# Rose-STL-Lab/spherical-dyffusion

Hardware: AMD Instinct MI355X
Metric: forecast-steps/sec (180x360, 63ch), 25-member ensemble DYffusion sampling, whole job (higher is better)
Workload: dtype f32 tensors; every GEMM-class kernel (1x1 convs, fused MLP, Legendre analysis/synthesis, dhconv) as 3-pass split-f16 MFMA with f32 accumulation; FFT / norms / pointwise in f32 (statistics f64); 1 GPU; 25-member ensemble x horizon-6 DYffusion sampling pass (6 forecaster + 10 interpolator SFNO forwards, dropout stream on, AR feedback), 180x360, 63 state + 2 forcing channels, embed 256, 8 blocks; horizon=6, relayed_members=0, parallelism=members of one initial condition sharded over GPUs, no data-path collective

## Files before the change

spherical-dyffusion_amd/csrc/common.h:

```cpp
#pragma once
#include <hip/hip_runtime.h>
#include <stdint.h>
#include <atomic>
#include <cmath>
#include <type_traits>

#include "../../include/sdy_amd.h"

#define SDY_HIP_TRY(expr)                       \
  do {                                          \
    hipError_t _e = (expr);                     \
    if (_e != hipSuccess) return (int)_e;       \
  } while (0)

#define SDY_TRY(expr)             \
  do {                            \
    int _r = (expr);              \
    if (_r != SDY_OK) return _r;  \
  } while (0)

static inline int sdy_launch_status() {
  hipError_t e = hipGetLastError();
  return e == hipSuccess ? SDY_OK : (int)e;
}

constexpr int SDY_MAX_DEVICES = 64;
static inline int sdy_current_device(int* dev) {
  SDY_HIP_TRY(hipGetDevice(dev));
  return (*dev >= 0 && *dev < SDY_MAX_DEVICES) ? SDY_OK : SDY_ERR_ARG;
}
inline int sdy_cu_count(int* n_cu) {
  static std::atomic<int> cache[SDY_MAX_DEVICES] = {};
  int dev = 0;
  SDY_TRY(sdy_current_device(&dev));
  int v = cache[dev].load(std::memory_order_relaxed);
  if (!v) {
    SDY_HIP_TRY(hipDeviceGetAttribute(&v, hipDeviceAttributeMultiprocessorCount, dev));
    cache[dev].store(v, std::memory_order_relaxed);
  }
  *n_cu = v;
  return SDY_OK;
}
int sdy_flags_ptr(unsigned** flags);
enum { SDY_RANGE_CONV = 0, SDY_RANGE_MLP = 1, SDY_RANGE_DHCONV = 2, SDY_RANGE_LEG_ANALYSIS = 3, SDY_RANGE_LEG_SYNTHESIS = 4 };
int sdy_headroom_ptr(int slot, unsigned** word);
struct SdyOncePerDevice {
  std::atomic<bool> done[SDY_MAX_DEVICES] = {};
  int slot(std::atomic<bool>** flag) {
    int dev = 0;
    SDY_TRY(sdy_current_device(&dev));
    *flag = &done[dev];
    return SDY_OK;
  }
};

constexpr int SDY_MAP_MAX = 128;
struct SdyImgMap {
  int on;
  unsigned char idx[SDY_MAP_MAX];
};
__host__ __device__ __forceinline__ int sdy_img(const SdyImgMap& m, int j) { return m.on ? (int)m.idx[j] : j; }
static inline int sdy_img_map_fill(SdyImgMap& m, const unsigned char* rows, int n) {
  m.on = 0;
  for (int i = 0; i < SDY_MAP_MAX; ++i) m.idx[i] = 0;
  if (!rows) return SDY_OK;
  if (n > SDY_MAP_MAX) return SDY_ERR_UNSUPPORTED;
  m.on = 1;
  for (int i = 0; i < n; ++i) m.idx[i] = rows[i];
  return SDY_OK;
}

typedef float f32x4 __attribute__((ext_vector_type(4)));
template <int B, int E, class F>
__device__ __forceinline__ void sdy_static_for(F&& f) {
  if constexpr (B < E) {
    f(std::integral_constant<int, B>{});
    sdy_static_for<B + 1, E>(f);
  }
}
typedef float sdy_f32x2 __attribute__((ext_vector_type(2)));
typedef _Float16 sdy_f16x2 __attribute__((ext_vector_type(2)));
typedef _Float16 sdy_f16x8 __attribute__((ext_vector_type(8)));
__device__ __forceinline__ void sdy_split8(const float* v, sdy_f16x8& hi, sdy_f16x8& lo) {
#pragma unroll
  for (int e = 0; e < 8; e += 2) {
    const sdy_f32x2 x = {v[e], v[e + 1]};
    const sdy_f16x2 h = __builtin_convertvector(x, sdy_f16x2);
    const sdy_f32x2 r = x - __builtin_convertvector(h, sdy_f32x2);
    const sdy_f16x2 l = __builtin_convertvector(r, sdy_f16x2);
    hi[e] = h[0]; hi[e + 1] = h[1];
    lo[e] = l[0]; lo[e + 1] = l[1];
  }
}
__device__ __forceinline__ void sdy_split8(const float* v, sdy_f16x8& hi, sdy_f16x8& lo, float& amax) {
#pragma unroll
  for (int e = 0; e < 8; e += 2) amax = __builtin_fmaxf(amax, __builtin_fmaxf(__builtin_fabsf(v[e]), __builtin_fabsf(v[e + 1])));
  sdy_split8(v, hi, lo);
}
#ifndef SDY_ACT_SX
#define SDY_ACT_SX 16.0f
#endif
constexpr int SDY_GROUP = 2 * 64;
static inline float sdy_h3_absmax(const float* w, size_t n) {
  float mx = 0.f;
  for (size_t i = 0; i < n; ++i) mx = std::fmax(mx, std::fabs(w[i]));
  return mx;
}
static inline float sdy_h3_scale(float absmax) {
  if (!(absmax > 0.f) || !std::isfinite(absmax)) return 1.0f;
  int e;
  std::frexp(absmax, &e);
  return std::ldexp(1.0f, 13 - e);
}
static inline void sdy_h3_split(float v, _Float16& hi, _Float16& lo) {
// ... 229 lines not shown
```

spherical-dyffusion_amd/csrc/conv_h3.hip:

```cpp
#include <cmath>
#include <cstdlib>
#include <type_traits>
#include <vector>

#include "common.h"

namespace {

constexpr int CE = 256;
constexpr int CTN = 64;
constexpr int CKMAX = 384;
constexpr int CRING = 4;
constexpr float CSX = SDY_ACT_SX;
constexpr int CSTAT_BYTES = CE * 2 * 8;
#ifndef SDY_CONV_STAMP_T0
#define SDY_CONV_STAMP_T0 2
#endif

template <int KBLK, int NW>
struct ConvCfg {
  static_assert(NW == 4 || NW == 8, "4 or 8 waves");
  static constexpr int NT = 64 * NW;
  static constexpr int MT = 8 / NW;
  static constexpr int RS = 4 * NW;
  static constexpr int OC = (8 * KBLK + RS - 1) / RS;
  static constexpr int RPT = 64 / NW;
  static constexpr int PPI = (8 * OC + RPT - 1) / RPT;
  static constexpr int KROW = KBLK <= 4 ? 256 : 384;
  static constexpr int KSW = KROW / 16;
  static constexpr int GPK = 4 * MT;
  static constexpr int GPW = MT * KSW;
  static constexpr int WGS = NW == 4 ? 2 : 1;
  static constexpr int TILE_BYTES = 2 * CTN * KROW * 2;
  static constexpr int LDS_BYTES = TILE_BYTES + CSTAT_BYTES + CE * 4 + SDY_GELU_TAB_BYTES;
};
#ifndef SDY_CONV_GELU_TAB
#define SDY_CONV_GELU_TAB 1
#endif

struct ConvParams {
  const float* x; long x_bs;
  const float* pa; const float* pd;
  const sdy_f16x8* w;
  const float* bias;
  const float* add; long add_bs; int add_mode;
  int act;
  float* out; long out_bs;
  int out_tiled;
  double* stats;
  int HW, B;
  int Cin;
  float out_scale;
  unsigned* flags;
  unsigned* head;
  const float* gelu_tab;
  SdyImgMap xmap;
  unsigned long long* stamps;
};

__device__ __forceinline__ int cv_swz(int px) { return (px & 15) ^ (((px >> 4) & 1) * 3); }
template <int KROW>
__device__ __forceinline__ int cv_off(int px, int c) { return px * KROW + (((c & ~15) | ((c ^ cv_swz(px)) & 15)) << 3); }

template <int KBLK, int NW, bool WS = false>
__global__ __launch_bounds__(64 * NW, NW == 4 ? 2 : 1) void conv_h3_kernel(const ConvParams p) {
  using G = ConvCfg<KBLK, NW>;
  static_assert(!WS || (KBLK == 4 && NW == 8), "weight-stationary: 256 input channels on 8 waves");
  constexpr int RING = WS ? G::KSW : CRING;
  constexpr int CMT = G::MT, CRS = G::RS, COC = G::OC, CRPT = G::RPT, KROW = G::KROW, CGPK = G::GPK, CGPW = G::GPW;
  __shared__ __attribute__((aligned(16))) unsigned char smem[G::LDS_BYTES];
  _Float16* Xs_hi = reinterpret_cast<_Float16*>(smem);
  _Float16* Xs_lo = Xs_hi + CTN * KROW;
  float* Os = reinterpret_cast<float*>(smem);

  const int tid = threadIdx.x, lane = tid & 63, wave = tid >> 6;
  auto Cin = [&] { return WS ? CE : p.Cin; };
  auto add_mode = [&] { return WS ? 1 : p.add_mode; };
  auto act = [&] { return WS ? 1 : p.act; };
  int h = lane >> 5, l31 = lane & 31;
  int q0 = tid & 15, o0 = tid >> 4;
  const int tpi = (p.HW + CTN - 1) / CTN;
  const int ntiles = tpi * p.B;
  const int t_per = (ntiles + (int)gridDim.x - 1) / (int)gridDim.x;
  const int t_begin = (int)blockIdx.x * t_per;
  const int t_end = (t_begin + t_per < ntiles) ? t_begin + t_per : ntiles;

  sdy_f16x8 r_hi[RING], r_lo[RING];
  constexpr int CGROUP_BYTES = SDY_GROUP * (int)sizeof(sdy_f16x8);
  const int uwave = __builtin_amdgcn_readfirstlane(wave);
  const char* const wbase = reinterpret_cast<const char*>(p.w) +
                            (WS ? (size_t)((uwave >> 1) * 2 * G::KSW + (uwave & 1)) * CGROUP_BYTES : (size_t)uwave * CGPW * CGROUP_BYTES);
  unsigned woff = (unsigned)lane * 16u;
#pragma unroll
  for (int s = 0; s < RING; ++s) {
    r_hi[s] = sdy_ring_ld(wbase, woff, 0);
    r_lo[s] = sdy_ring_ld(wbase, woff, CGROUP_BYTES / 2);
    woff += (WS ? 2 : 1) * CGROUP_BYTES;
  }
  constexpr int NWIN = KBLK * CMT;
  if (!WS && NWIN == 1) woff -= CRING * CGROUP_BYTES;

  double* Ss = reinterpret_cast<double*>(smem + G::TILE_BYTES);
  float* Bs = reinterpret_cast<float*>(smem + G::TILE_BYTES + CSTAT_BYTES);
  if (tid < CE) {
    Bs[tid] = p.bias ? p.bias[tid] / p.out_scale : 0.0f;
    Ss[2 * tid] = 0.0; Ss[2 * tid + 1] = 0.0;
  }
  float* Gt = reinterpret_cast<float*>(smem + G::TILE_BYTES + CSTAT_BYTES + CE * 4);
  const unsigned gt_base = (unsigned)(uintptr_t)Gt;
  const bool tab_gelu = SDY_CONV_GELU_TAB && act() == 1;
  if (tab_gelu) gelu_tab_to_lds(Gt, p.gelu_tab, tid, G::NT, 1.0f / SDY_GELU_SX);
  const float os_scale = tab_gelu ? p.out_scale * SDY_GELU_WS : p.out_scale;

  f32x4 xr[COC][8], addv[CRPT];
  auto img = [&](const float* base, long bs, int t) { return base + (long)(t / tpi) * bs; };
  auto ximg = [&](int t) { return p.x + (long)sdy_img(p.xmap, t / tpi) * p.x_bs; };
  auto lane_col = [&](int t) {
    const int nn = (t % tpi) * CTN + 4 * q0;
    return nn < p.HW ? nn : 0;
  };
  const float* addsrc = p.add ? p.add : p.out;
  const long addsrc_bs = p.add ? p.add_bs : p.out_bs;
  if (t_begin < t_end) {
    const float* xz = ximg(t_begin);
    const unsigned xo = (unsigned)(8 * o0 * p.HW + lane_col(t_begin)) * 4u;
#pragma unroll
    for (int oc = 0; oc < COC; ++oc)
#pragma unroll
      for (int e = 0; e < 8; ++e) {
        const int ch = 8 * (o0 + CRS * oc) + e;
        xr[oc][e] = f32x4{0.f, 0.f, 0.f, 0.f};
        if (WS || ch < Cin()) xr[oc][e] = sdy_ld16s(xz + (long)(8 * CRS * oc + e) * p.HW, xo);
      }
  }

  for (int tile = t_begin; tile < t_end; ++tile) {
    asm volatile("" : "+v"(l31), "+v"(h), "+v"(q0), "+v"(o0));
    const int tile_it = tile - t_begin;
    auto stamp = [&](int i) {
      if (SDY_STAMPS_ON && p.stamps && blockIdx.x == 3 && tid == 0 && tile_it >= SDY_CONV_STAMP_T0 && tile_it < SDY_CONV_STAMP_T0 + 4)
        p.stamps[(tile_it - SDY_CONV_STAMP_T0) * 8 + i] = __builtin_amdgcn_s_memtime();
    };
    stamp(0);
    const int z = tile / tpi;
    const int zx = sdy_img(p.xmap, z);
    const int n0 = (tile - z * tpi) * CTN;
    const bool full = n0 + CTN <= p.HW;

    {
      float amax = 0.0f;
      const bool ok = full || (n0 + 4 * q0 < p.HW);
#pragma unroll
      for (int oc = 0; oc < COC; ++oc) {
        const int c0 = 8 * (o0 + CRS * oc);
        if (8 * CRS * oc + 8 * CRS > KROW && c0 >= KROW) continue;
        float av[8], dv[8];
        if (p.pa) {
          const f32x4 a0 = *reinterpret_cast<const f32x4*>(p.pa + (long)zx * CE + c0);
          const f32x4 a1 = *reinterpret_cast<const f32x4*>(p.pa + (long)zx * CE + c0 + 4);
          const f32x4 d0 = *reinterpret_cast<const f32x4*>(p.pd + (long)zx * CE + c0);
          const f32x4 d1 = *reinterpret_cast<const f32x4*>(p.pd + (long)zx * CE + c0 + 4);
#pragma unroll
          for (int e = 0; e < 4; ++e) {
            av[e] = a0[e] * CSX; av[e + 4] = a1[e] * CSX;
            dv[e] = d0[e] * CSX; dv[e + 4] = d1[e] * CSX;
          }
        } else {
#pragma unroll
          for (int e = 0; e < 8; ++e) { av[e] = CSX; dv[e] = 0.f; }
        }
#pragma unroll
        for (int pp = 0; pp < 4; ++pp) {
          sdy_f16x8 vh, vl;
          float v[8];
#pragma unroll
          for (int e = 0; e < 8; ++e) v[e] = (ok && (WS || c0 + e < Cin())) ? fmaf(xr[oc][e][pp], av[e], dv[e]) : 0.0f;
          sdy_split8(v, vh, vl, amax);
          const int off = cv_off<KROW>(4 * q0 + pp, o0 + CRS * oc);
          *reinterpret_cast<sdy_f16x8*>(Xs_hi + off) = vh;
          *reinterpret_cast<sdy_f16x8*>(Xs_lo + off) = vl;
        }
      }
      sdy_flag_range(p.flags, amax, p.head);
    }
    __syncthreads();
    stamp(1);
    const int col = n0 + 4 * q0;
    const bool c_ok = full || col < p.HW;
    const unsigned ro = (unsigned)(o0 * p.HW + (c_ok ? col : 0)) * 4u;
    const unsigned ro_out = p.out_tiled ? (unsigned)(o0 * CTN + 4 * q0) * 4u : ro;
    const int out_rs = p.out_tiled ? CTN : p.HW;
    const int tnext = (tile + 1 < t_end) ? tile + 1 : tile;
    const float* xz_next = ximg(tnext);
    const unsigned xo_next = (unsigned)(8 * o0 * p.HW + lane_col(tnext)) * 4u;
    if constexpr (WS) {
      const float* az = img(p.add, p.add_bs, tile);
#pragma unroll
      for (int i = 0; i < CRPT; ++i) addv[i] = sdy_ld16s(az + (long)(CRS * i) * p.HW, ro);
      __builtin_amdgcn_sched_barrier(0);
    }
    stamp(2);
    f32x16 acc[CMT][2];
#pragma unroll
    for (int mi = 0; mi < CMT; ++mi)
#pragma unroll
      for (int r4 = 0; r4 < 4; ++r4) {
        const f32x4 b4 = *reinterpret_cast<const f32x4*>(Bs + 32 * (CMT * wave + mi) + 8 * r4 + 4 * h);
#pragma unroll
        for (int j = 0; j < 2; ++j)
#pragma unroll
          for (int r = 0; r < 4; ++r) acc[mi][j][4 * r4 + r] = b4[r];
      }
    auto ld_b = [&](int ks, sdy_f16x8* bh, sdy_f16x8* bl) {
#pragma unroll
      for (int j = 0; j < 2; ++j) {
        const int off = cv_off<KROW>(32 * j + l31, 2 * ks + h);
        bh[j] = *reinterpret_cast<const sdy_f16x8*>(Xs_hi + off);
        bl[j] = *reinterpret_cast<const sdy_f16x8*>(Xs_lo + off);
      }
    };
    if constexpr (WS) {
      sdy_f16x8 bh[2][2], bl[2][2];
      ld_b(0, bh[0], bl[0]);
      sdy_static_for<0, G::KSW>([&](auto ks_c) {
        constexpr int ks = decltype(ks_c)::value, c = ks & 1;
        if constexpr (ks + 1 < G::KSW) ld_b(ks + 1, bh[c ^ 1], bl[c ^ 1]);
#pragma unroll
        for (int j = 0; j < 2; ++j) SDY_CROSS_TERM(acc[0][j] = __builtin_amdgcn_mfma_f32_32x32x16_f16(r_lo[ks], bh[c][j], acc[0][j], 0, 0, 0));
#pragma unroll
        for (int j = 0; j < 2; ++j) SDY_CROSS_TERM(acc[0][j] = __builtin_amdgcn_mfma_f32_32x32x16_f16(r_hi[ks], bl[c][j], acc[0][j], 0, 0, 0));
#pragma unroll
        for (int j = 0; j < 2; ++j) acc[0][j] = __builtin_amdgcn_mfma_f32_32x32x16_f16(r_hi[ks], bh[c][j], acc[0][j], 0, 0, 0);
        __builtin_amdgcn_sched_barrier(0);
      });
    } else {
#pragma unroll
    for (int kb = 0; kb < KBLK; ++kb) {
#pragma unroll
      for (int i = 0; i < 4; ++i) {
        const int ks = 4 * kb + i;
        sdy_f16x8 bh[2], bl[2];
        ld_b(ks, bh, bl);
#pragma unroll
        for (int mi = 0; mi < CMT; ++mi) {
          const int g = kb * CGPK + CMT * i + mi;
          const int s = g % CRING;
#pragma unroll
          for (int j = 0; j < 2; ++j) SDY_CROSS_TERM(acc[mi][j] = __builtin_amdgcn_mfma_f32_32x32x16_f16(r_lo[s], bh[j], acc[mi][j], 0, 0, 0));
#pragma unroll
          for (int j = 0; j < 2; ++j) SDY_CROSS_TERM(acc[mi][j] = __builtin_amdgcn_mfma_f32_32x32x16_f16(r_hi[s], bl[j], acc[mi][j], 0, 0, 0));
#pragma unroll
          for (int j = 0; j < 2; ++j) acc[mi][j] = __builtin_amdgcn_mfma_f32_32x32x16_f16(r_hi[s], bh[j], acc[mi][j], 0, 0, 0);
          r_hi[s] = sdy_ring_ld(wbase, woff, 0);
          r_lo[s] = sdy_ring_ld(wbase, woff, CGROUP_BYTES / 2);
          woff += CGROUP_BYTES;
          if ((g + CRING + 1) % (NWIN * CRING) == 0) woff -= NWIN * CRING * CGROUP_BYTES;
          __builtin_amdgcn_sched_barrier(0);
        }
      }
    }
    }

    stamp(3);
    if constexpr (WS) {
      static_assert(!WS || COC == 1, "one channel octet per thread");
#pragma unroll
      for (int e = 0; e < 8; ++e) xr[0][e] = sdy_ld16s(xz_next + (long)e * p.HW, xo_next);
      __builtin_amdgcn_sched_barrier(0);
    } else {
      const float* az = img(addsrc, addsrc_bs, tile);
#pragma unroll
      for (int i = 0; i < CRPT; ++i) addv[i] = p.add ? sdy_ld16s(az + (long)(CRS * i) * p.HW, ro) : f32x4{0.f, 0.f, 0.f, 0.f};
    }
    __syncthreads();
    stamp(4);
#pragma unroll
    for (int mi = 0; mi < CMT; ++mi)
#pragma unroll
      for (int j = 0; j < 2; ++j)
#pragma unroll
        for (int r = 0; r < 16; ++r) {
          const int row = 32 * (CMT * wave + mi) + (r & 3) + 8 * (r >> 2) + 4 * h;
          Os[row * CTN + 32 * j + l31] = acc[mi][j][r] * os_scale;
        }
    __syncthreads();
    stamp(5);
    {
      float* oz = p.out + (long)z * p.out_bs + (p.out_tiled ? (long)(tile - z * tpi) * (CE * CTN) : 0L);
#pragma unroll
      for (int i = 0; i < CRPT; ++i) {
        f32x4 v = *reinterpret_cast<const f32x4*>(Os + (o0 + CRS * i) * CTN + 4 * q0);
        if (tab_gelu) {
          if (add_mode() == 1) v = addv[i] * SDY_GELU_WS + v;
          v = f32x4{gelu_tab16(v.x, gt_base), gelu_tab16(v.y, gt_base), gelu_tab16(v.z, gt_base), gelu_tab16(v.w, gt_base)};
        } else {
        if (add_mode() == 1) v += addv[i];
        if (act() == 1) {
          const sdy_gf2 g0 = gelu_erf2(sdy_gf2{v.x, v.y}), g1 = gelu_erf2(sdy_gf2{v.z, v.w});
          v = f32x4{g0.x, g0.y, g1.x, g1.y};
        }
        }
        if (add_mode() == 2) v += addv[i];
        if (c_ok) sdy_st16s(oz + (long)(CRS * i) * out_rs, ro_out, v);
#pragma unroll
        for (int k = 0; k < G::PPI; ++k) {
          const int piece = G::PPI * i + k, oc = piece >> 3, e = piece & 7;
          if (oc < COC) {
            const int ch = 8 * (o0 + CRS * oc) + e;
            if constexpr (!WS)
              if (ch < Cin()) xr[oc][e] = sdy_ld16s(xz_next + (long)(8 * CRS * oc + e) * p.HW, xo_next);
          }
        }
        if (p.stats) {
          const float s1 = row16_sum(c_ok ? sdy_quad_sum(v) : 0.0f);
          const float s2 = row16_sum(c_ok ? sdy_quad_sumsq(v) : 0.0f);
          if (q0 == 0) {
            double* st = Ss + 2 * (o0 + CRS * i);
            __hip_atomic_fetch_add(st, (double)s1, __ATOMIC_RELAXED, __HIP_MEMORY_SCOPE_WORKGROUP);
            __hip_atomic_fetch_add(st + 1, (double)s2, __ATOMIC_RELAXED, __HIP_MEMORY_SCOPE_WORKGROUP);
          }
        }
      }
    }
    stamp(6);
    {
      const int nt = tile + 1;
      if (p.stats && (nt >= t_end || nt / tpi != z)) {
        __syncthreads();
        if (tid < CE) {
          double* st = p.stats + ((long)z * CE + tid) * 2;
          __hip_atomic_fetch_add(st, Ss[2 * tid], __ATOMIC_RELAXED, __HIP_MEMORY_SCOPE_AGENT);
          __hip_atomic_fetch_add(st + 1, Ss[2 * tid + 1], __ATOMIC_RELAXED, __HIP_MEMORY_SCOPE_AGENT);
          Ss[2 * tid] = 0.0; Ss[2 * tid + 1] = 0.0;
        }
      }
    }
    stamp(7);
    __syncthreads();
  }
}

}

#if SDY_STAMPS_ON
static unsigned long long* g_cstamps = nullptr;
SDY_DEBUG_EXPORT int sdy_conv256_h3_debug_stamps(unsigned long long* host64) {
  if (!g_cstamps || !host64) return SDY_ERR_STATE;
  SDY_HIP_TRY(hipDeviceSynchronize());
  SDY_HIP_TRY(hipMemcpy(host64, g_cstamps, 64 * sizeof(unsigned long long), hipMemcpyDeviceToHost));
  return SDY_OK;
}
#endif

extern "C" int sdy_conv256_h3_supported(int Cin, int Cout) { return (Cin >= 1 && Cin <= CKMAX && Cout == CE) ? 1 : 0; }

static void conv_layout(int Cin, int* nw, int* ksw, int* mt) {
  const int kblk = (Cin + 63) / 64;
  *nw = kblk <= 4 ? 4 : 8;
  *ksw = kblk <= 4 ? 16 : 24;
  *mt = 8 / *nw;
}

extern "C" size_t sdy_conv256_h3_pack_bytes_cin(int Cin) {
  int nw, ksw, mt;
  conv_layout(Cin < 1 ? 1 : Cin, &nw, &ksw, &mt);
  return (size_t)nw * mt * ksw * SDY_GROUP * sizeof(sdy_f16x8);
}
extern "C" size_t sdy_conv256_h3_pack_bytes(void) { return sdy_conv256_h3_pack_bytes_cin(CE); }

extern "C" int sdy_conv256_h3_pack_cin(const float* w_host, int Cin, void* dev, float* scale) {
  if (!w_host || !dev || !scale || Cin < 1 || Cin > CKMAX) return SDY_ERR_ARG;
  const float s = sdy_h3_scale(sdy_h3_absmax(w_host, (size_t)CE * Cin));
  int nw, ksw, mt;
  conv_layout(Cin, &nw, &ksw, &mt);
  const size_t gh = (size_t)SDY_GROUP * 8;
  std::vector<_Float16> buf((size_t)nw * mt * ksw * gh);
  _Float16* d = buf.data();
  for (int w = 0; w < nw; ++w)
    for (int ks = 0; ks < ksw; ++ks)
      for (int mi = 0; mi < mt; ++mi, d += gh)
        sdy_h3_put_group(d, s, [&](int r, int k) {
          const int kk = 16 * ks + k;
          return kk < Cin ? w_host[(size_t)(32 * (mt * w + mi) + r) * Cin + kk] : 0.0f;
        });
  SDY_HIP_TRY(hipMemcpy(dev, buf.data(), buf.size() * sizeof(_Float16), hipMemcpyHostToDevice));
  *scale = s;
  return SDY_OK;
}
extern "C" int sdy_conv256_h3_pack(const float* w_host, void* dev, float* scale) {
  return sdy_conv256_h3_pack_cin(w_host, CE, dev, scale);
}
// ... 59 lines not shown
```

spherical-dyffusion_amd/csrc/mlp_h3.hip:

```cpp
#include <cstdlib>
#include <vector>
#include <cmath>
#include <type_traits>

#include "common.h"

typedef const sdy_f16x8 __attribute__((address_space(1)))* wptr_t;
typedef _Float16 f16x4 __attribute__((ext_vector_type(4)));

namespace {

constexpr int ME = 256;
constexpr int MH = 512;
constexpr int TN = 64;
constexpr int HC = 128;
constexpr int NCH = MH / HC;
constexpr int KS1 = ME / 16;
constexpr int KSC = HC / 16;
constexpr int RING = 16;
constexpr int NGROUPS = NCH * 2 * RING;
static_assert(KS1 == RING && 2 * KSC == RING, "ring slot = index inside a block");
constexpr float SX = SDY_ACT_SX;

struct MlpParams {
// ... 41 lines not shown
  const int t_per = (ntiles + (int)gridDim.x - 1) / (int)gridDim.x;
  const int t_begin = (int)blockIdx.x * t_per;
  const int t_end = (t_begin + t_per < ntiles) ? t_begin + t_per : ntiles;
  int z = 0, zo = 0, n0 = 0;
  bool full = true;

  sdy_f16x8 r_hi[RING], r_lo[RING];
  auto wbase_of = [&](int ln) { return (wptr_t)(p.w + (size_t)wave * (NGROUPS + RING) * SDY_GROUP + ln); };
  wptr_t wp = wbase_of(lane);
#pragma unroll
  for (int s = 0; s < RING; ++s) {
    r_hi[s] = wp[s * SDY_GROUP];
    r_lo[s] = wp[s * SDY_GROUP + 64];
  }
  wp += RING * SDY_GROUP;

  int q0 = tid & 15, o0 = tid >> 4;
  f32x4 xr[2][8];
  const float* pf_base = nullptr;
  const float* res_base = nullptr;
  unsigned pf_off = 0u;
  int pf_rs = 0;
  auto prefetch_setup = [&](int t) {
    const int zz = t / tpi, nn = (t - zz * tpi) * TN;
    const bool ok = nn + 4 * q0 < p.HW;
    pf_base = p.x + (long)zz * p.x_bs + (p.x_tiled ? (long)(t - zz * tpi) * (ME * TN) : 0L);
    pf_rs = p.x_tiled ? TN : p.HW;
    pf_off = p.x_tiled ? (unsigned)(8 * o0 * TN + 4 * q0) * 4u : (unsigned)(8 * o0 * p.HW + (ok ? nn + 4 * q0 : 0)) * 4u;
  };
  auto prefetch_piece = [&](int piece) {
    const int oc = piece >> 3, e = piece & 7;
    xr[oc][e] = sdy_ld16s(pf_base + (long)(8 * 16 * oc + e) * pf_rs, pf_off);
  };
  auto prefetch_x = [&](int t) {
    const int zz = t / tpi, nn = (t - zz * tpi) * TN;
    const bool ok = nn + 4 * q0 < p.HW;
    const float* xz = p.x + (long)zz * p.x_bs + (p.x_tiled ? (long)(t - zz * tpi) * (ME * TN) : 0L);
    const int rs = p.x_tiled ? TN : p.HW;
    const unsigned xo = p.x_tiled ? (unsigned)(8 * o0 * TN + 4 * q0) * 4u : (unsigned)(8 * o0 * p.HW + (ok ? nn + 4 * q0 : 0)) * 4u;
#pragma unroll
    for (int oc = 0; oc < 2; ++oc)
#pragma unroll
      for (int e = 0; e < 8; ++e) xr[oc][e] = sdy_ld16s(xz + (long)(8 * 16 * oc + e) * rs, xo);
  };
  auto load_coeffs = [&](int zz) {
    const int t = 64 * wave + (int)__builtin_amdgcn_mbcnt_hi(~0u, __builtin_amdgcn_mbcnt_lo(~0u, 0u));
    const long c = (long)zz * ME + t, co = (long)sdy_img(p.omap, zz) * ME + t;
    Cf[t] = p.pa ? p.pa[c] * SX : SX;
    Cf[ME + t] = p.pa ? p.pd[c] * SX : 0.0f;
    Cf[2 * ME + t] = p.add_a ? p.add_a[co] : 1.0f;
    Cf[3 * ME + t] = p.add_a ? p.add_d[co] : 0.0f;
  };
  Cb2[tid] = DROP ? p.b2[tid] * p.drop_scale : p.b2[tid];
  if (t_begin < t_end) load_coeffs(t_begin / tpi);
  __syncthreads();
  if (t_begin < t_end) prefetch_x(t_begin);
  double psum[16], psq[16];
#pragma unroll
  for (int i = 0; i < 16; ++i) { psum[i] = 0.0; psq[i] = 0.0; }

  for (int tile = t_begin; tile < t_end; ++tile) {
  asm volatile("" : "+v"(l31), "+v"(h), "+v"(q0), "+v"(o0));
  const int tile_it = tile - t_begin;
  auto stamp = [&](int i) {
#if SDY_STAMPS_ON
    if (p.stamps && blockIdx.x == 3 && tid == 0 && tile_it >= 2 && tile_it < 6)
      p.stamps[(tile_it - 2) * 16 + i] = __builtin_amdgcn_s_memtime();
#else
    (void)i; (void)tile_it;
    if (p.stamps && tid == 0) asm volatile("s_nop 0");
#endif
  };
  stamp(0);
  z = tile / tpi;
  zo = sdy_img(p.omap, z);
  n0 = (tile - z * tpi) * TN;
  full = n0 + TN <= p.HW;

  auto stage_x = [&](auto full_t) {
    constexpr bool kFull = decltype(full_t)::value;
    float amax = 0.0f;
    const bool ok = kFull || (n0 + 4 * q0 < p.HW);
#pragma unroll
    for (int oc = 0; oc < 2; ++oc) {
      float av[8], dv[8];
      {
        const int c0 = 8 * (o0 + 16 * oc);
        const f32x4 a0 = *reinterpret_cast<const f32x4*>(Cf + c0), a1 = *reinterpret_cast<const f32x4*>(Cf + c0 + 4);
        const f32x4 d0 = *reinterpret_cast<const f32x4*>(Cf + ME + c0), d1 = *reinterpret_cast<const f32x4*>(Cf + ME + c0 + 4);
#pragma unroll
        for (int e = 0; e < 4; ++e) { av[e] = a0[e]; av[e + 4] = a1[e]; dv[e] = d0[e]; dv[e + 4] = d1[e]; }
      }
#pragma unroll
      for (int pp = 0; pp < 4; ++pp) {
        const int px = 4 * q0 + pp;
        sdy_f16x8 vh, vl;
        float v[8];
#pragma unroll
        for (int e = 0; e < 8; ++e) v[e] = (kFull || ok) ? fmaf(xr[oc][e][pp], av[e], dv[e]) : 0.0f;
        sdy_split8(v, vh, vl, amax);
        const int off = xs_off(px, o0 + 16 * oc);
        *reinterpret_cast<sdy_f16x8*>(Xs_hi + off) = vh;
        *reinterpret_cast<sdy_f16x8*>(Xs_lo + off) = vl;
      }
    }
    sdy_flag_range(p.flags, amax, p.head);
  };
  if (full) stage_x(std::true_type{});
  else stage_x(std::false_type{});
  __syncthreads();

  f32x16 oacc[2][2];
  f32x4 rres[16];
  const int e_col = n0 + 4 * (tid & 15);
  const bool e_ok = full || e_col < p.HW;
  const unsigned e_ro = (unsigned)((tid >> 4) * p.HW + (e_ok ? e_col : 0)) * 4u;

  constexpr bool do_drop = DROP;
  const int zq = zo / p.rows_per_call, zt = zo - zq * p.rows_per_call;
  const uint32_t call_z = p.call + (uint32_t)zq;
  const uint32_t c1_base = (uint32_t)(((uint64_t)(zt + p.batch_offset) * (uint64_t)(MH >> 2)) & 0xFFFFFFFFu);

  f32x16 acc[2];
  f32x4 bv[4];
  auto load_bias = [&](int hc) {
    const int row0 = HC * hc + 32 * wave + 4 * h;
#pragma unroll
    for (int g4 = 0; g4 < 4; ++g4) bv[g4] = *reinterpret_cast<const f32x4*>(p.b1 + row0 + 8 * g4);
// ... 429 lines not shown
          const int i0 = 2 * (4 * mi + g4);
          rres[i0] = sdy_ld16s(res_base + (long)(16 * i0) * p.HW, e_ro);
          rres[i0 + 1] = sdy_ld16s(res_base + (long)(16 * (i0 + 1)) * p.HW, e_ro);
          prefetch_piece(i0);
          prefetch_piece(i0 + 1);
        }
      }
    }
    stamp(13);
    __syncthreads();
    stamp(14);
    if (e_ok) {
      float* oz = p.out + (long)zo * p.out_bs;
      const float* os = Os + (tid >> 4) * TN + 4 * (tid & 15);
#pragma unroll
      for (int i = 0; i < 16; ++i) {
        const int row = (tid >> 4) + 16 * i;
        f32x4 v = *reinterpret_cast<const f32x4*>(os + 16 * i * TN);
        if (p.add) v += rres[i] * Cf[2 * ME + row] + Cf[3 * ME + row];
        sdy_st16s(oz + (long)(16 * i) * p.HW, e_ro, v);
        if (p.stats) {
          psum[i] += (double)sdy_quad_sum(v);
          psq[i] += (double)sdy_quad_sumsq(v);
        }
      }
    }
    if (p.stats) {
      const int nt = tile + 1;
      if (nt >= t_end || nt / tpi != z) {
#pragma unroll
        for (int i = 0; i < 16; ++i) {
          double s1 = psum[i], s2 = psq[i];
#pragma unroll
          for (int m = 1; m < 16; m <<= 1) {
            s1 += __shfl_xor(s1, m, 64);
            s2 += __shfl_xor(s2, m, 64);
          }
          if ((tid & 15) == 0) {
            double* st = p.stats + ((long)zo * ME + (tid >> 4) + 16 * i) * 2;
            __hip_atomic_fetch_add(st, s1, __ATOMIC_RELAXED, __HIP_MEMORY_SCOPE_AGENT);
            __hip_atomic_fetch_add(st + 1, s2, __ATOMIC_RELAXED, __HIP_MEMORY_SCOPE_AGENT);
          }
          psum[i] = 0.0; psq[i] = 0.0;
        }
      }
    }
  }
  stamp(15);
  __syncthreads();
  {
    const int nt = tile + 1;
    if (nt < t_end && nt / tpi != z) {
      load_coeffs(nt / tpi);
      __syncthreads();
    }
  }
  }
}

}

#ifndef SDY_MLP_INJECT_TU
#if SDY_STAMPS_ON
static unsigned long long* g_stamps = nullptr;
SDY_DEBUG_EXPORT int sdy_mlp_h3_debug_stamps(unsigned long long* host64) {
  if (!g_stamps || !host64) return SDY_ERR_STATE;
  SDY_HIP_TRY(hipDeviceSynchronize());
  SDY_HIP_TRY(hipMemcpy(host64, g_stamps, 64 * sizeof(unsigned long long), hipMemcpyDeviceToHost));
  return SDY_OK;
}
#endif

extern "C" int sdy_mlp_h3_supported(int E, int hidden) { return (E == ME && hidden == MH) ? 1 : 0; }

extern "C" size_t sdy_mlp_h3_pack_bytes(int E, int hidden) {
  if (!sdy_mlp_h3_supported(E, hidden)) return 0;
  return (size_t)4 * (NGROUPS + RING) * SDY_GROUP * sizeof(sdy_f16x8);
}

extern "C" int sdy_mlp_h3_pack(const float* w1_host, const float* w2_host, int E, int hidden, void* packed_dev,
                               float* scale1, float* scale2) {
  if (!w1_host || !w2_host || !packed_dev || !scale1 || !scale2) return SDY_ERR_ARG;
  if (!sdy_mlp_h3_supported(E, hidden)) return SDY_ERR_UNSUPPORTED;
  const float s1 = sdy_h3_scale(sdy_h3_absmax(w1_host, (size_t)E * hidden));
  const float s2 = sdy_h3_scale(sdy_h3_absmax(w2_host, (size_t)E * hidden));
  const size_t gh = (size_t)SDY_GROUP * 8;
  std::vector<_Float16> buf((size_t)4 * (NGROUPS + RING) * gh, (_Float16)0.0f);
  for (int w = 0; w < 4; ++w) {
    _Float16* d = buf.data() + (size_t)w * (NGROUPS + RING) * gh;
    auto put_fc1 = [&](int hc) {
      for (int ks = 0; ks < KS1; ++ks, d += gh) {
        const float* blk = w1_host + (size_t)(128 * hc + 32 * w) * ME + 16 * ks;
        sdy_h3_put_group(d, s1, [&](int r, int k) { return blk[(size_t)r * ME + k]; });
      }
    };
    auto put_fc2 = [&](int hc) {
      for (int t = 0; t < KSC; ++t)
        for (int mi = 0; mi < 2; ++mi, d += gh) {
          const float* blk = w2_host + (size_t)(64 * w + 32 * mi) * MH + 16 * (KSC * hc + t);
          sdy_h3_put_group(d, s2, [&](int r, int k) { return blk[(size_t)r * MH + k]; });
        }
    };
    put_fc1(0);
    put_fc1(1);
    for (int hc = 1; hc < NCH; ++hc) {
      put_fc2(hc - 1);
// ... 98 lines not shown
```

spherical-dyffusion_amd/ops.py:

```python
from __future__ import annotations

import ctypes as C
from typing import Optional

import torch

from ._lib import SdyConvArgs, SdyMlpArgs, SdyPairArgs, aligned, check, current_stream, lib, ptr


def _f32c(t: torch.Tensor) -> torch.Tensor:
    if not t.is_cuda:
        raise RuntimeError("sdy_amd ops run on the GPU only (no CPU fallback)")
    return aligned(t.to(torch.float32).contiguous())


def _aux(t: torch.Tensor, dev) -> torch.Tensor:
    return t.detach().to(dev, torch.float32).contiguous()


def contract_dhconv(x: torch.Tensor, weight: torch.Tensor, separable: bool = False,
                    operator_type: str = "dhconv", gemm_mode: Optional[str] = None) -> torch.Tensor:
    if separable or operator_type != "dhconv":
        raise NotImplementedError("only the non-separable dhconv contraction is on the hot path")
    B, Ci, L, M = x.shape
# ... 112 lines not shown
    if stats is not None:
        assert stats.dtype == torch.float64 and stats.is_cuda and stats.is_contiguous() and stats.numel() == B * Cout * 2
        a.stats = ptr(stats)
    if batch_scale is not None:
        bs = _aux(batch_scale, x.device)
        a.batch_scale = ptr(bs)
        keep.append(bs)
    with torch.cuda.device(x.device):
        check(lib.sdy_conv1x1(C.byref(a), current_stream()), "sdy_conv1x1")
    return out


def pack_conv256(weight: torch.Tensor, device):
    w = weight.detach().to("cpu", torch.float32).reshape(weight.shape[0], -1).contiguous()
    if not lib.sdy_conv256_h3_supported(w.shape[1], w.shape[0]):
        raise NotImplementedError("the persistent conv kernel needs 256 output and at most 384 input channels")
    buf = torch.empty(lib.sdy_conv256_h3_pack_bytes_cin(w.shape[1]), dtype=torch.uint8, device=device)
    sc = C.c_float()
    with torch.cuda.device(device):
        check(lib.sdy_conv256_h3_pack_cin(ptr(w), w.shape[1], ptr(buf), C.byref(sc)), "sdy_conv256_h3_pack_cin")
    return buf, sc.value


def pack_h3(weight: torch.Tensor, device):
    w = weight.detach().to("cpu", torch.float32).reshape(weight.shape[0], -1).contiguous()
    Cout, Cin = w.shape
    nbytes = lib.sdy_h3_pack_bytes(Cout, Cin)
    buf = torch.empty(nbytes, dtype=torch.uint8, device=device)
    sc = C.c_float()
    with torch.cuda.device(device):
        check(lib.sdy_h3_pack_weight(ptr(w), Cout, Cin, ptr(buf), C.byref(sc)), "sdy_h3_pack_weight")
    return buf, sc.value


def pack_mlp_h3(w1: torch.Tensor, w2: torch.Tensor, device):
    a = w1.detach().to("cpu", torch.float32).reshape(w1.shape[0], -1).contiguous()
    b = w2.detach().to("cpu", torch.float32).reshape(w2.shape[0], -1).contiguous()
    hidden, E = a.shape
    assert b.shape == (E, hidden)
    if not lib.sdy_mlp_h3_supported(E, hidden):
        raise NotImplementedError(f"fused MLP kernel supports E=256, hidden=512 (got {E}, {hidden}); use conv1x1")
    buf = torch.empty(lib.sdy_mlp_h3_pack_bytes(E, hidden), dtype=torch.uint8, device=device)
    s1, s2 = C.c_float(), C.c_float()
    with torch.cuda.device(device):
        check(lib.sdy_mlp_h3_pack(ptr(a), ptr(b), E, hidden, ptr(buf), C.byref(s1), C.byref(s2)), "sdy_mlp_h3_pack")
    return (buf, s1.value, s2.value)


def mlp_fused(x: torch.Tensor, w1: torch.Tensor, b1: torch.Tensor, w2: torch.Tensor, b2: torch.Tensor, *,
              pre_affine=None, add: Optional[torch.Tensor] = None, drop_p: float = 0.0, seed: int = 0, call: int = 0,
              stream_fc1: int = 0, stream_fc2: int = 1, batch_offset: int = 0,
              batch_scale: Optional[torch.Tensor] = None, out: Optional[torch.Tensor] = None,
              prepared=None, add_affine=None, stats: Optional[torch.Tensor] = None,
              keep_masks=None) -> torch.Tensor:
    x = _f32c(x)
    B, E, H, W = x.shape
    if prepared is None:
        prepared = pack_mlp_h3(w1, w2, x.device)
    hidden = b1.numel()
    if out is None:
        out = torch.empty_like(x)
    a = SdyMlpArgs()
    a.x, a.x_bstride = ptr(x), E * H * W
    a.w, a.w1_scale, a.w2_scale = ptr(prepared[0]), prepared[1], prepared[2]
    bb1, bb2 = _aux(b1, x.device), _aux(b2, x.device)
    a.b1, a.b2 = ptr(bb1), ptr(bb2)
    a.out, a.out_bstride = ptr(out), E * H * W
    keep = [x, bb1, bb2, out, prepared]
    if pre_affine is not None:
        pa, pd = _aux(pre_affine[0], x.device), _aux(pre_affine[1], x.device)
        a.pa, a.pd = ptr(pa), ptr(pd)
        keep += [pa, pd]
    if add is not None:
        ad = _aux(add, x.device)
        a.add, a.add_bstride = ptr(ad), E * H * W
        keep.append(ad)
        if add_affine is not None:
            ra, rd = _aux(add_affine[0], x.device), _aux(add_affine[1], x.device)
            a.add_a, a.add_d = ptr(ra), ptr(rd)
            keep += [ra, rd]
    a.B, a.E, a.hidden, a.HW = B, E, hidden, H * W
    a.drop_p = drop_p
    a.seed, a.call, a.stream_fc1, a.stream_fc2, a.batch_offset = seed, call, stream_fc1, stream_fc2, batch_offset
    if batch_scale is not None:
        bs = _aux(batch_scale, x.device)
        a.batch_scale = ptr(bs)
        keep.append(bs)
    if stats is not None:
        assert stats.dtype == torch.float64 and stats.is_cuda and stats.is_contiguous() and stats.numel() == B * E * 2
        a.stats = ptr(stats)
    if keep_masks is not None:
        kh, ko = _aux(keep_masks[0], x.device), _aux(keep_masks[1], x.device)
        assert kh.numel() == B * hidden * H * W and ko.numel() == B * E * H * W
        a.keep_hidden, a.keep_out = ptr(kh), ptr(ko)
        keep += [kh, ko]
    with torch.cuda.device(x.device):
        check(lib.sdy_mlp_h3(C.byref(a), current_stream()), "sdy_mlp_h3")
    return out


def pack_pair_h3(w1: torch.Tensor, w2: torch.Tensor, device):
    a = w1.detach().to("cpu", torch.float32).reshape(w1.shape[0], -1).contiguous()
    b = w2.detach().to("cpu", torch.float32).reshape(w2.shape[0], -1).contiguous()
    hidden, Cin = a.shape
    Cout = b.shape[0]
    assert b.shape == (Cout, hidden)
    if not lib.sdy_pair_h3_supported(Cin, hidden, Cout):
        raise NotImplementedError(f"fused conv pair supports hidden=256 with (Cin<=144, Cout=256) or (Cin<=416, Cout<=64); "
                                  f"got {Cin}->{hidden}->{Cout}; use conv1x1 twice")
    buf = torch.empty(lib.sdy_pair_h3_pack_bytes(Cin, hidden, Cout), dtype=torch.uint8, device=device)
    s1, s2 = C.c_float(), C.c_float()
    with torch.cuda.device(device):
        check(lib.sdy_pair_h3_pack(ptr(a), ptr(b), Cin, hidden, Cout, ptr(buf), C.byref(s1), C.byref(s2)), "sdy_pair_h3_pack")
    return (buf, s1.value, s2.value)


def conv_pair(x: torch.Tensor, w1: torch.Tensor, b1: Optional[torch.Tensor], w2: torch.Tensor, *,
              add: Optional[torch.Tensor] = None, out: Optional[torch.Tensor] = None, prepared=None,
              stats: Optional[torch.Tensor] = None) -> torch.Tensor:
    x = _f32c(x)
    B, Cin, H, W = x.shape
    if prepared is None:
        prepared = pack_pair_h3(w1, w2, x.device)
    hidden, Cout = w1.shape[0], w2.shape[0]
    if out is None:
        out = torch.empty(B, Cout, H, W, dtype=torch.float32, device=x.device)
    a = SdyPairArgs()
    a.x, a.x_bstride = ptr(x), Cin * H * W
    a.w, a.w1_scale, a.w2_scale = ptr(prepared[0]), prepared[1], prepared[2]
    keep = [x, out, prepared]
    if b1 is not None:
        bb1 = _aux(b1, x.device)
        a.b1 = ptr(bb1)
        keep.append(bb1)
    a.out, a.out_bstride = ptr(out), Cout * H * W
    if add is not None:
        ad = _aux(add, x.device)
        a.add, a.add_bstride = ptr(ad), (0 if ad.shape[0] == 1 and B > 1 else Cout * H * W)
        keep.append(ad)
    a.B, a.Cin, a.hidden, a.Cout, a.HW = B, Cin, hidden, Cout, H * W
    if stats is not None:
        assert stats.dtype == torch.float64 and stats.is_cuda and stats.is_contiguous() and stats.numel() == B * Cout * 2
        a.stats = ptr(stats)
    with torch.cuda.device(x.device):
        check(lib.sdy_pair_h3(C.byref(a), current_stream()), "sdy_pair_h3")
    return out
# ... 173 lines not shown
```

Baseline: 169.8 member-forecast-steps/s.

## Stage per-image affine coefficients in LDS and track tile indices incrementally in conv

In the weight-stationary 1x1 conv kernel, the per-image pre-affine scale and shift are now loaded into shared memory once per image instead of being read from global memory on every tile. Image and tile indices are advanced incrementally with uniform (readfirstlane) map lookups instead of per-tile division and modulo. Partial-tile stores become unconditional, using shuffled copies of a valid lane so out-of-range lanes repeat an in-bounds write. The MLP kernel hoists its output-row map lookup to image boundaries, and the Python wrapper gains out_rows/add_by_launch_row plumbing. This uses extra LDS and adds a sync at image boundaries, and the new Python arguments depend on struct fields not shown here.

Result: no change. 170.0 member-forecast-steps/s (median of 6 runs) (+0.1%).

```diff
diff --git a/spherical-dyffusion_amd/csrc/common.h b/spherical-dyffusion_amd/csrc/common.h
--- a/spherical-dyffusion_amd/csrc/common.h
+++ b/spherical-dyffusion_amd/csrc/common.h
@@ -60,6 +60,13 @@
   unsigned char idx[SDY_MAP_MAX];
 };
 __host__ __device__ __forceinline__ int sdy_img(const SdyImgMap& m, int j) { return m.on ? (int)m.idx[j] : j; }
+__device__ __forceinline__ int sdy_img_uniform(const SdyImgMap& m, int j) {
+  if (!m.on) return j;
+  const int ju = __builtin_amdgcn_readfirstlane(j);
+  unsigned w;
+  __builtin_memcpy(&w, __builtin_assume_aligned(m.idx + (ju & ~3), 4), 4);
+  return (int)((w >> (8 * (ju & 3))) & 255u);
+}
 static inline int sdy_img_map_fill(SdyImgMap& m, const unsigned char* rows, int n) {
   m.on = 0;
   for (int i = 0; i < SDY_MAP_MAX; ++i) m.idx[i] = 0;
diff --git a/spherical-dyffusion_amd/csrc/conv_h3.hip b/spherical-dyffusion_amd/csrc/conv_h3.hip
--- a/spherical-dyffusion_amd/csrc/conv_h3.hip
+++ b/spherical-dyffusion_amd/csrc/conv_h3.hip
@@ -33,6 +33,7 @@
   static constexpr int WGS = NW == 4 ? 2 : 1;
   static constexpr int TILE_BYTES = 2 * CTN * KROW * 2;
   static constexpr int LDS_BYTES = TILE_BYTES + CSTAT_BYTES + CE * 4 + SDY_GELU_TAB_BYTES;
+  static constexpr int COEF_BYTES = 2 * CE * 4;
 };
 #ifndef SDY_CONV_GELU_TAB
 #define SDY_CONV_GELU_TAB 1
@@ -68,7 +69,7 @@
   static_assert(!WS || (KBLK == 4 && NW == 8), "weight-stationary: 256 input channels on 8 waves");
   constexpr int RING = WS ? G::KSW : CRING;
   constexpr int CMT = G::MT, CRS = G::RS, COC = G::OC, CRPT = G::RPT, KROW = G::KROW, CGPK = G::GPK, CGPW = G::GPW;
-  __shared__ __attribute__((aligned(16))) unsigned char smem[G::LDS_BYTES];
+  __shared__ __attribute__((aligned(16))) unsigned char smem[G::LDS_BYTES + (WS ? G::COEF_BYTES : 0)];
   _Float16* Xs_hi = reinterpret_cast<_Float16*>(smem);
   _Float16* Xs_lo = Xs_hi + CTN * KROW;
   float* Os = reinterpret_cast<float*>(smem);
@@ -111,19 +112,30 @@
   const bool tab_gelu = SDY_CONV_GELU_TAB && act() == 1;
   if (tab_gelu) gelu_tab_to_lds(Gt, p.gelu_tab, tid, G::NT, 1.0f / SDY_GELU_SX);
   const float os_scale = tab_gelu ? p.out_scale * SDY_GELU_WS : p.out_scale;
+  float* Cf = reinterpret_cast<float*>(smem + G::LDS_BYTES);
+  auto load_coeffs = [&](int zz) {
+    if constexpr (WS) {
+      if (tid < CE) {
+        Cf[tid] = p.pa ? p.pa[(long)zz * CE + tid] * CSX : CSX;
+        Cf[CE + tid] = p.pa ? p.pd[(long)zz * CE + tid] * CSX : 0.0f;
+      }
+    }
+  };
+  const int t_first = t_begin < t_end ? t_begin : 0;
+  int z = __builtin_amdgcn_readfirstlane(t_first / tpi), ti = t_first - z * tpi;
+  int zx = sdy_img_uniform(p.xmap, z);
+  load_coeffs(zx);
 
   f32x4 xr[COC][8], addv[CRPT];
-  auto img = [&](const float* base, long bs, int t) { return base + (long)(t / tpi) * bs; };
-  auto ximg = [&](int t) { return p.x + (long)sdy_img(p.xmap, t / tpi) * p.x_bs; };
-  auto lane_col = [&](int t) {
-    const int nn = (t % tpi) * CTN + 4 * q0;
+  auto lane_col = [&](int t_img) {
+    const int nn = t_img * CTN + 4 * q0;
     return nn < p.HW ? nn : 0;
   };
   const float* addsrc = p.add ? p.add : p.out;
   const long addsrc_bs = p.add ? p.add_bs : p.out_bs;
   if (t_begin < t_end) {
-    const float* xz = ximg(t_begin);
-    const unsigned xo = (unsigned)(8 * o0 * p.HW + lane_col(t_begin)) * 4u;
+    const float* xz = p.x + (long)zx * p.x_bs;
+    const unsigned xo = (unsigned)(8 * o0 * p.HW + lane_col(ti)) * 4u;
 #pragma unroll
     for (int oc = 0; oc < COC; ++oc)
 #pragma unroll
@@ -132,6 +144,10 @@
         xr[oc][e] = f32x4{0.f, 0.f, 0.f, 0.f};
         if (WS || ch < Cin()) xr[oc][e] = sdy_ld16s(xz + (long)(8 * CRS * oc + e) * p.HW, xo);
       }
+  }
+  if constexpr (WS) {
+    __builtin_amdgcn_s_waitcnt(0x0F70);
+    __syncthreads();
   }
 
   for (int tile = t_begin; tile < t_end; ++tile) {
@@ -142,9 +158,7 @@
         p.stamps[(tile_it - SDY_CONV_STAMP_T0) * 8 + i] = __builtin_amdgcn_s_memtime();
     };
     stamp(0);
-    const int z = tile / tpi;
-    const int zx = sdy_img(p.xmap, z);
-    const int n0 = (tile - z * tpi) * CTN;
+    const int n0 = ti * CTN;
     const bool full = n0 + CTN <= p.HW;
 
     {
@@ -155,7 +169,12 @@
         const int c0 = 8 * (o0 + CRS * oc);
         if (8 * CRS * oc + 8 * CRS > KROW && c0 >= KROW) continue;
         float av[8], dv[8];
-        if (p.pa) {
+        if constexpr (WS) {
+          const f32x4 a0 = *reinterpret_cast<const f32x4*>(Cf + c0), a1 = *reinterpret_cast<const f32x4*>(Cf + c0 + 4);
+          const f32x4 d0 = *reinterpret_cast<const f32x4*>(Cf + CE + c0), d1 = *reinterpret_cast<const f32x4*>(Cf + CE + c0 + 4);
+#pragma unroll
+          for (int e = 0; e < 4; ++e) { av[e] = a0[e]; av[e + 4] = a1[e]; dv[e] = d0[e]; dv[e + 4] = d1[e]; }
+        } else if (p.pa) {
           const f32x4 a0 = *reinterpret_cast<const f32x4*>(p.pa + (long)zx * CE + c0);
           const f32x4 a1 = *reinterpret_cast<const f32x4*>(p.pa + (long)zx * CE + c0 + 4);
           const f32x4 d0 = *reinterpret_cast<const f32x4*>(p.pd + (long)zx * CE + c0);
@@ -187,14 +206,20 @@
     stamp(1);
     const int col = n0 + 4 * q0;
     const bool c_ok = full || col < p.HW;
-    const unsigned ro = (unsigned)(o0 * p.HW + (c_ok ? col : 0)) * 4u;
-    const unsigned ro_out = p.out_tiled ? (unsigned)(o0 * CTN + 4 * q0) * 4u : ro;
+    const unsigned ro = (unsigned)(o0 * p.HW + (c_ok ? col : WS ? n0 : 0)) * 4u;
+    const unsigned ro_out = p.out_tiled ? (unsigned)(o0 * CTN + ((!WS || c_ok) ? 4 * q0 : 0)) * 4u : ro;
     const int out_rs = p.out_tiled ? CTN : p.HW;
-    const int tnext = (tile + 1 < t_end) ? tile + 1 : tile;
-    const float* xz_next = ximg(tnext);
-    const unsigned xo_next = (unsigned)(8 * o0 * p.HW + lane_col(tnext)) * 4u;
+    const bool has_next = tile + 1 < t_end;
+    int z_next = z, ti_next = ti, zx_next = zx;
+    if (has_next && ++ti_next == tpi) {
+      ti_next = 0;
+      z_next = z + 1;
+      zx_next = sdy_img_uniform(p.xmap, z_next);
+    }
+    const float* xz_next = p.x + (long)zx_next * p.x_bs;
+    const unsigned xo_next = (unsigned)(8 * o0 * p.HW + lane_col(ti_next)) * 4u;
     if constexpr (WS) {
-      const float* az = img(p.add, p.add_bs, tile);
+      const float* az = p.add + (long)z * p.add_bs;
 #pragma unroll
       for (int i = 0; i < CRPT; ++i) addv[i] = sdy_ld16s(az + (long)(CRS * i) * p.HW, ro);
       __builtin_amdgcn_sched_barrier(0);
@@ -268,7 +293,7 @@
       for (int e = 0; e < 8; ++e) xr[0][e] = sdy_ld16s(xz_next + (long)e * p.HW, xo_next);
       __builtin_amdgcn_sched_barrier(0);
     } else {
-      const float* az = img(addsrc, addsrc_bs, tile);
+      const float* az = addsrc + (long)z * addsrc_bs;
 #pragma unroll
       for (int i = 0; i < CRPT; ++i) addv[i] = p.add ? sdy_ld16s(az + (long)(CRS * i) * p.HW, ro) : f32x4{0.f, 0.f, 0.f, 0.f};
     }
@@ -286,7 +311,7 @@
     __syncthreads();
     stamp(5);
     {
-      float* oz = p.out + (long)z * p.out_bs + (p.out_tiled ? (long)(tile - z * tpi) * (CE * CTN) : 0L);
+      float* oz = p.out + (long)z * p.out_bs + (p.out_tiled ? (long)ti * (CE * CTN) : 0L);
 #pragma unroll
       for (int i = 0; i < CRPT; ++i) {
         f32x4 v = *reinterpret_cast<const f32x4*>(Os + (o0 + CRS * i) * CTN + 4 * q0);
@@ -301,7 +326,17 @@
         }
         }
         if (add_mode() == 2) v += addv[i];
-        if (c_ok) sdy_st16s(oz + (long)(CRS * i) * out_rs, ro_out, v);
+        if constexpr (WS) {
+          f32x4 vs = v;
+          if (!full) {
+            const int l0 = lane & ~15;
+            const f32x4 v0 = f32x4{__shfl(v.x, l0, 64), __shfl(v.y, l0, 64), __shfl(v.z, l0, 64), __shfl(v.w, l0, 64)};
+            vs = c_ok ? v : v0;
+          }
+          sdy_st16s(oz + (long)(CRS * i) * out_rs, ro_out, vs);
+        } else {
+          if (c_ok) sdy_st16s(oz + (long)(CRS * i) * out_rs, ro_out, v);
+        }
 #pragma unroll
         for (int k = 0; k < G::PPI; ++k) {
           const int piece = G::PPI * i + k, oc = piece >> 3, e = piece & 7;
@@ -323,9 +358,8 @@
       }
     }
     stamp(6);
-    {
-      const int nt = tile + 1;
-      if (p.stats && (nt >= t_end || nt / tpi != z)) {
+    if (!has_next || z_next != z) {
+      if (p.stats) {
         __syncthreads();
         if (tid < CE) {
           double* st = p.stats + ((long)z * CE + tid) * 2;
@@ -334,9 +368,11 @@
           Ss[2 * tid] = 0.0; Ss[2 * tid + 1] = 0.0;
         }
       }
+      if (has_next) load_coeffs(zx_next);
     }
     stamp(7);
     __syncthreads();
+    z = z_next; ti = ti_next; zx = zx_next;
   }
 }
 
diff --git a/spherical-dyffusion_amd/csrc/mlp_h3.hip b/spherical-dyffusion_amd/csrc/mlp_h3.hip
--- a/spherical-dyffusion_amd/csrc/mlp_h3.hip
+++ b/spherical-dyffusion_amd/csrc/mlp_h3.hip
@@ -117,7 +117,10 @@
     Cf[3 * ME + t] = p.add_a ? p.add_d[co] : 0.0f;
   };
   Cb2[tid] = DROP ? p.b2[tid] * p.drop_scale : p.b2[tid];
-  if (t_begin < t_end) load_coeffs(t_begin / tpi);
+  if (t_begin < t_end) {
+    load_coeffs(t_begin / tpi);
+    zo = sdy_img(p.omap, t_begin / tpi);
+  }
   __syncthreads();
   if (t_begin < t_end) prefetch_x(t_begin);
   double psum[16], psq[16];
@@ -138,7 +141,6 @@
   };
   stamp(0);
   z = tile / tpi;
-  zo = sdy_img(p.omap, z);
   n0 = (tile - z * tpi) * TN;
   full = n0 + TN <= p.HW;
 
@@ -674,6 +676,7 @@
     const int nt = tile + 1;
     if (nt < t_end && nt / tpi != z) {
       load_coeffs(nt / tpi);
+      zo = sdy_img(p.omap, nt / tpi);
       __syncthreads();
     }
   }
diff --git a/spherical-dyffusion_amd/ops.py b/spherical-dyffusion_amd/ops.py
--- a/spherical-dyffusion_amd/ops.py
+++ b/spherical-dyffusion_amd/ops.py
@@ -188,9 +188,20 @@
               stream_fc1: int = 0, stream_fc2: int = 1, batch_offset: int = 0,
               batch_scale: Optional[torch.Tensor] = None, out: Optional[torch.Tensor] = None,
               prepared=None, add_affine=None, stats: Optional[torch.Tensor] = None,
-              keep_masks=None) -> torch.Tensor:
+              keep_masks=None, out_rows=None, add_by_launch_row: bool = False) -> torch.Tensor:
     x = _f32c(x)
     B, E, H, W = x.shape
+    rows_host = None
+    if out_rows is not None:
+        assert add is not None and len(out_rows) == B and (out is not None or not add_by_launch_row)
+        n_rows = out.shape[0] if out is not None else add.shape[0]
+        assert all(0 <= int(r) < n_rows for r in out_rows)
+        rows_host = (C.c_ubyte * B)(*[int(r) for r in out_rows])
+        if out is None:
+            out = torch.zeros(n_rows, E, H, W, dtype=torch.float32, device=x.device)
+    else:
+        assert not add_by_launch_row
+        n_rows = B
     if prepared is None:
         prepared = pack_mlp_h3(w1, w2, x.device)
     hidden = b1.numel()
@@ -216,6 +227,9 @@
             a.add_a, a.add_d = ptr(ra), ptr(rd)
             keep += [ra, rd]
     a.B, a.E, a.hidden, a.HW = B, E, hidden, H * W
+    if rows_host is not None:
+        a.out_rows, a.rows_per_call = C.addressof(rows_host), n_rows
+        a.add_by_launch_row = 1 if add_by_launch_row else 0
     a.drop_p = drop_p
     a.seed, a.call, a.stream_fc1, a.stream_fc2, a.batch_offset = seed, call, stream_fc1, stream_fc2, batch_offset
     if batch_scale is not None:
@@ -223,11 +237,11 @@
         a.batch_scale = ptr(bs)
         keep.append(bs)
     if stats is not None:
-        assert stats.dtype == torch.float64 and stats.is_cuda and stats.is_contiguous() and stats.numel() == B * E * 2
+        assert stats.dtype == torch.float64 and stats.is_cuda and stats.is_contiguous() and stats.numel() == n_rows * E * 2
         a.stats = ptr(stats)
     if keep_masks is not None:
         kh, ko = _aux(keep_masks[0], x.device), _aux(keep_masks[1], x.device)
-        assert kh.numel() == B * hidden * H * W and ko.numel() == B * E * H * W
+        assert kh.numel() == n_rows * hidden * H * W and ko.numel() == n_rows * E * H * W
         a.keep_hidden, a.keep_out = ptr(kh), ptr(ko)
         keep += [kh, ko]
     with torch.cuda.device(x.device):
```
